# chrischoy/DeepGlobalRegistration

Measured on AMD Instinct MI355X. Metric: pair registrations/sec (FCGF x2 + 1-NN + 6-D inlier net + gate + weighted Procrustes + SE(3) refinement), higher is better.
Workload: dtype f32 results via 2 x f16 split operands (3 f16 MFMA products per MAC, f32 accumulate); k = 1 convs, kNN re-evaluation and registration in exact f32, SVD in f64

## Files before the change

deepglobalregistration_amd/csrc/knn_prefilter.h:

```cpp
#pragma once
#include "knn_common.h"

typedef __attribute__((ext_vector_type(8))) short bf16x8;
typedef __attribute__((ext_vector_type(16))) float f32x16_t;
constexpr float KNN_TAU_C = 8e-5f;
constexpr int KNN_ST = 4;
constexpr int KNN_SLOTS = 32;
#ifndef DGR_KNN_SUB
#define DGR_KNN_SUB 2
#endif
constexpr int KNN_SUB = DGR_KNN_SUB;

__device__ __forceinline__ unsigned short knn_f2bf(float x) {
  uint32_t u = __float_as_uint(x);
  if ((u & 0x7f800000u) == 0x7f800000u) return (unsigned short)((u >> 16) | ((u & 0xffffu) ? 0x40u : 0u));
  u += 0x7fffu + ((u >> 16) & 1u);
  return (unsigned short)(u >> 16);
}
__device__ __forceinline__ float knn_bf2f(unsigned short h) { return __uint_as_float((uint32_t)h << 16); }
__device__ __forceinline__ uint32_t knn_ord(float f) {
  const uint32_t u = __float_as_uint(f);
  return u ^ ((u >> 31) ? 0xffffffffu : 0x80000000u);
}
__device__ __forceinline__ float knn_unord(uint32_t k) {
  return __uint_as_float(k ^ ((k >> 31) ? 0x80000000u : 0xffffffffu));
}
__device__ __forceinline__ int knn_acc_slot(int e, int h) { return (e & 3) + 8 * (e >> 2) + 4 * h; }

template <bool TOPK>
__device__ __forceinline__ int64_t knn_slot_row(int s, int t, int n_tiles) {
  return (int64_t)(TOPK ? (s + t) & 31 : s) * n_tiles + t;
}
template <bool TOPK>
__global__ void __launch_bounds__(256)
    knn_pack_kernel(const float *__restrict__ F0, const float *__restrict__ F1, KnnBatch B,
                    bf16x8 *__restrict__ Qp, bf16x8 *__restrict__ Rp, float *__restrict__ na, float *__restrict__ nb,
                    uint32_t *__restrict__ nb_max, int32_t *__restrict__ fallback) {
  const int pair = blockIdx.y >> 1, side = blockIdx.y & 1;
  const KnnPair d = B.p[pair];
  const int64_t N = side ? d.n1 : d.n0;
  const int64_t n_pad = (N + 31) / 32 * 32;
  const int64_t t = (int64_t)blockIdx.x * blockDim.x + threadIdx.x;
  int64_t row = t >> 2;
  if (row >= n_pad) return;
// ... 9 lines not shown
  for (int e = 0; e < 8; ++e) { hi[e] = 0; lo[e] = 0; }
  if (row < N) {
    const float *src = F + row * 32 + 16 * ch + 8 * g;
    const float4 v0 = *reinterpret_cast<const float4 *>(src), v1 = *reinterpret_cast<const float4 *>(src + 4);
    const float x[8] = {v0.x, v0.y, v0.z, v0.w, v1.x, v1.y, v1.z, v1.w};
#pragma unroll
    for (int e = 0; e < 8; ++e) {
      if (!(fabsf(x[e]) < 1e18f)) fallback[pair] = 1;
      const unsigned short h = knn_f2bf(x[e]);
      const unsigned short l = knn_f2bf(x[e] - knn_bf2f(h));
      hi[e] = (short)knn_f2bf(knn_bf2f(h) * scale);
      lo[e] = (short)knn_f2bf(knn_bf2f(l) * scale);
    }
  }
  const int64_t tile = prow >> 5;
  const int r = (int)(prow & 31);
  packed[(tile * 4 + ch) * 64 + r + 32 * g] = hi;
  packed[(tile * 4 + 2 + ch) * 64 + r + 32 * g] = lo;
  float n = 0.f;
  if (row < N) {
    const float *src = F + row * 32 + 16 * ch + 8 * g;
#pragma unroll
    for (int e = 0; e < 8; ++e) n = fmaf(src[e], src[e], n);
  }
  n += __shfl_xor(n, 1, 64);
  n += __shfl_xor(n, 2, 64);
  if (g == 0 && ch == 0) {
    if (row >= N) n = side ? __builtin_inff() : 0.f;
    else if (side) atomicMax(nb_max + pair, __float_as_uint(n));
    norms[prow] = n;
  }
}

template <bool PASS2, bool TOPK>
__global__ void __launch_bounds__(256, 2)
    knn_mfma_kernel(const bf16x8 *__restrict__ Qp, const bf16x8 *__restrict__ Rp, const float *__restrict__ nbp,
                    KnnBatch B, int splits, int sub_arg, int64_t q_begin, int64_t span, uint32_t *__restrict__ mt,
                    const float *__restrict__ nap, const uint32_t *__restrict__ nb_max,
                    const float *__restrict__ thr_q, int32_t *__restrict__ cand, int32_t *__restrict__ cand_cnt,
                    int slots_arg) {
  __shared__ bf16x8 sA[2][KNN_ST * 4 * 64];
  __shared__ __attribute__((aligned(16))) float sNb[2][KNN_ST * 32];
  const int sub = TOPK ? sub_arg : KNN_SUB, slots = TOPK ? slots_arg : KNN_SLOTS;
  constexpr int NM = TOPK ? 16 : 1;
  const KnnPair d = B.p[blockIdx.z];
  const int n_qblocks = (d.n0 + 31) >> 5, n_rtiles = (d.n1 + 31) >> 5;
  if ((int)blockIdx.x * 16 >= n_qblocks) return;
  const int64_t N0 = d.n0, N1 = d.n1;
  const bf16x8 *Q = Qp + (int64_t)d.qb0 * 256, *R = Rp + (int64_t)d.rt0 * 256;
  const float *nb = nbp + (int64_t)d.rt0 * 32;
  const int64_t qrow0 = d.q0 - q_begin;
  mt += qrow0;
  cand += qrow0 * slots;
  cand_cnt += qrow0;
  const int tid = threadIdx.x;
  const int lane = tid & 63;
  const int wave = __builtin_amdgcn_readfirstlane(tid >> 6);
  const int h = lane >> 5;
  const int qb0 = (blockIdx.x * 4 + wave) * 4;
  bf16x8 bq[4][4];
  float m[4][NM], thr[4];
#pragma unroll
  for (int u = 0; u < 4; ++u) {
    const int qb = min(qb0 + u, n_qblocks - 1);
#pragma unroll
    for (int f = 0; f < 4; ++f) bq[u][f] = Q[((int64_t)qb * 4 + f) * 64 + lane];
#pragma unroll
    for (int e = 0; e < NM; ++e) m[u][e] = __builtin_inff();
    thr[u] = 0.f;
    if constexpr (PASS2) {
      const int64_t q = (int64_t)qb * 32 + (lane & 31);
      const bool live = q < N0 && qb0 + u < n_qblocks;
      if constexpr (TOPK) {
        thr[u] = live ? thr_q[qrow0 + q] : -__builtin_inff();
      } else {
        const float nmax = __uint_as_float(nb_max[blockIdx.z]);
        thr[u] = live ? knn_unord(mt[q]) + KNN_TAU_C * (nap[(int64_t)d.qb0 * 32 + q] + nmax) : -__builtin_inff();
      }
    }
  }
  const int n_stages = (n_rtiles + KNN_ST - 1) / KNN_ST;
  const int sps = (n_stages + splits - 1) / splits;
  const int s_begin = blockIdx.y * sps, s_end = min(n_stages, s_begin + sps);
  const int step = PASS2 ? 1 : sub;
  const int s_first = PASS2 ? s_begin : s_begin + min((int)(blockIdx.y % sub), max(s_end - s_begin - 1, 0));
  if (s_first >= s_end) return;
  bf16x8 pre[KNN_ST];
  float pre_nb = 0.f;
  auto request = [&](int t0) {
#pragma unroll
    for (int j = 0; j < KNN_ST; ++j) pre[j] = R[(int64_t)min(t0 + j, n_rtiles - 1) * 256 + tid];
    if (tid < KNN_ST * 32) pre_nb = nb[(int64_t)min(t0 + (tid >> 5), n_rtiles - 1) * 32 + (tid & 31)];
  };
  auto deposit = [&](int buf) {
#pragma unroll
    for (int j = 0; j < KNN_ST; ++j) sA[buf][j * 256 + tid] = pre[j];
    if (tid < KNN_ST * 32) sNb[buf][tid] = pre_nb;
  };
  request(s_first * KNN_ST);
  deposit(0);
  __syncthreads();
  int buf = 0;
  for (int st = s_first; st < s_end; st += step) {
    const int t0 = st * KNN_ST;
    if (st + step < s_end) request((st + step) * KNN_ST);
#pragma unroll
    for (int j = 0; j < KNN_ST; ++j) {
      const int t = t0 + j;
      if (t >= n_rtiles) break;
      const bf16x8 a0 = sA[buf][(j * 4 + 0) * 64 + lane], a1 = sA[buf][(j * 4 + 1) * 64 + lane];
      const bf16x8 a2 = sA[buf][(j * 4 + 2) * 64 + lane], a3 = sA[buf][(j * 4 + 3) * 64 + lane];
      f32x16_t c0;
#pragma unroll
      for (int g = 0; g < 4; ++g) {
        const float4 v = *reinterpret_cast<const float4 *>(&sNb[buf][j * 32 + 8 * g + 4 * h]);
        c0[4 * g] = v.x; c0[4 * g + 1] = v.y; c0[4 * g + 2] = v.z; c0[4 * g + 3] = v.w;
      }
      f32x16_t acc[4];
#pragma unroll
      for (int u = 0; u < 4; ++u) acc[u] = __builtin_amdgcn_mfma_f32_32x32x16_bf16(a0, bq[u][0], c0, 0, 0, 0);
#pragma unroll
      for (int u = 0; u < 4; ++u) acc[u] = __builtin_amdgcn_mfma_f32_32x32x16_bf16(a1, bq[u][1], acc[u], 0, 0, 0);
#pragma unroll
      for (int u = 0; u < 4; ++u) acc[u] = __builtin_amdgcn_mfma_f32_32x32x16_bf16(a0, bq[u][2], acc[u], 0, 0, 0);
#pragma unroll
      for (int u = 0; u < 4; ++u) acc[u] = __builtin_amdgcn_mfma_f32_32x32x16_bf16(a1, bq[u][3], acc[u], 0, 0, 0);
#pragma unroll
      for (int u = 0; u < 4; ++u) acc[u] = __builtin_amdgcn_mfma_f32_32x32x16_bf16(a2, bq[u][0], acc[u], 0, 0, 0);
#pragma unroll
      for (int u = 0; u < 4; ++u) acc[u] = __builtin_amdgcn_mfma_f32_32x32x16_bf16(a3, bq[u][1], acc[u], 0, 0, 0);
#pragma unroll
      for (int u = 0; u < 4; ++u) {
        if constexpr (!PASS2 && TOPK) {
#pragma unroll
          for (int e = 0; e < 16; ++e) m[u][e] = fminf(m[u][e], acc[u][e]);
        } else {
          float bm = fminf(fminf(acc[u][0], acc[u][1]), fminf(acc[u][2], acc[u][3]));
#pragma unroll
          for (int e = 4; e < 16; e += 4)
            bm = fminf(bm, fminf(fminf(acc[u][e], acc[u][e + 1]), fminf(acc[u][e + 2], acc[u][e + 3])));
          if constexpr (!PASS2) {
            m[u][0] = fminf(m[u][0], bm);
          } else if (!(bm > thr[u])) {
            const int64_t q = (int64_t)(qb0 + u) * 32 + (lane & 31);
#pragma unroll
            for (int e = 0; e < 16; ++e) {
              const int64_t i = knn_slot_row<TOPK>(knn_acc_slot(e, h), t, n_rtiles);
              if (!(acc[u][e] > thr[u]) && q < N0 && i < N1 && qb0 + u < n_qblocks) {
                const int slot = atomicAdd(cand_cnt + q, 1);
                if (slot < slots) cand[q * slots + slot] = (int32_t)(i + d.r0);
              }
            }
          }
        }
      }
    }
    if (st + step < s_end) deposit(buf ^ 1);
    __syncthreads();
    buf ^= 1;
  }
  if constexpr (!PASS2) {
#pragma unroll
    for (int u = 0; u < 4; ++u) {
      const int64_t q = (int64_t)(qb0 + u) * 32 + (lane & 31);
      const bool live = qb0 + u < n_qblocks && q < N0;
      if constexpr (TOPK) {
        if (live) {
#pragma unroll
          for (int e = 0; e < 16; ++e)
            atomicMin(mt + (int64_t)knn_acc_slot(e, h) * span + q, knn_ord(m[u][e]));
        }
      } else {
        const float mm = fminf(m[u][0], __shfl_xor(m[u][0], 32, 64));
        if (lane < 32 && live) atomicMin(mt + q, knn_ord(mm));
      }
    }
  }
}

struct KnnPlan {
  int64_t q_begin, span, n0_max;
  int qb_max, rt_max;
  int qgroups_all;
  bf16x8 *Qp, *Rp;
  float *na, *nb;
  uint32_t *mt;
  float *thr;
  int32_t *qlist, *cand_cnt, *cand;
  uint32_t *nb_max;
  int32_t *fallback, *qcount, *flags;
};

template <bool TOPK>
inline int knn_prefilter_setup(dgr_ctx *ctx, const float *F0, const float *F1, KnnBatch &B, int slots,
                               hipStream_t stream, KnnPlan *plan) {
  KnnPlan &P = *plan;
  DgrArena &arena = ctx->arena;
  int n_qb = 0, n_rt = 0;
  P.qb_max = P.rt_max = P.qgroups_all = 0;
  for (int p = 0; p < B.np; ++p) {
    KnnPair &d = B.p[p];
    d.qb0 = n_qb;
    d.rt0 = n_rt;
    const int qb = (d.n0 + 31) / 32, rt = (d.n1 + 31) / 32;
    n_qb += qb;
    n_rt += rt;
    P.qb_max = std::max(P.qb_max, qb);
    P.rt_max = std::max(P.rt_max, rt);
    P.qgroups_all += (int)dgr_ceil_div(qb, 16);
  }
  P.n0_max = knn_n0_max(B);
  P.span = knn_query_span(B, &P.q_begin);
  const int64_t n_mt = (TOPK ? 32 : 1) * P.span;
  DGR_ALLOC(P.Qp, arena, bf16x8, (int64_t)n_qb * 256);
  DGR_ALLOC(P.Rp, arena, bf16x8, (int64_t)n_rt * 256);
  DGR_ALLOC(P.na, arena, float, (int64_t)n_qb * 32);
  DGR_ALLOC(P.nb, arena, float, (int64_t)n_rt * 32);
  DGR_ALLOC(P.mt, arena, uint32_t, n_mt);
  P.thr = nullptr;
  if (TOPK) DGR_ALLOC(P.thr, arena, float, P.span);
  DGR_ALLOC(P.qlist, arena, int32_t, P.span);
  DGR_ALLOC(P.cand_cnt, arena, int32_t, P.span + 4 * KNN_MAXP);
  DGR_ALLOC(P.cand, arena, int32_t, P.span * slots);
  int32_t *pair_words = P.cand_cnt + P.span;
  P.nb_max = reinterpret_cast<uint32_t *>(pair_words);
  P.fallback = pair_words + KNN_MAXP;
  P.qcount = pair_words + 2 * KNN_MAXP;
  P.flags = pair_words + 3 * KNN_MAXP;
  DGR_HIP_CHECK(hipMemsetAsync(P.cand_cnt, 0, (size_t)(P.span + 4 * KNN_MAXP) * sizeof(int32_t), stream));
  DGR_HIP_CHECK(hipMemsetAsync(P.mt, 0xff, (size_t)n_mt * sizeof(uint32_t), stream));
  dim3 grid((unsigned)dgr_ceil_div((int64_t)std::max(P.qb_max, P.rt_max) * 32 * 4, 256), 2 * B.np);
  knn_pack_kernel<TOPK><<<grid, 256, 0, stream>>>(F0, F1, B, P.Qp, P.Rp, P.na, P.nb, P.nb_max, P.fallback);
  DGR_LAUNCH_CHECK();
  return DGR_OK;
}

template <bool PASS2, bool TOPK>
inline int knn_mfma_launch(dgr_ctx *ctx, const KnnBatch &B, const KnnPlan &P, int sub, int slots, hipStream_t stream) {
  const auto kernel = knn_mfma_kernel<PASS2, TOPK>;
  static int per_cu = 0;
  if (per_cu == 0) {
    int n = 0;
    DGR_HIP_CHECK(hipOccupancyMaxActiveBlocksPerMultiprocessor(&n, kernel, 256, 0));
    per_cu = n < 1 ? 1 : n;
  }
  const int capacity = ctx->num_cus * per_cu;
  const int stages = (int)dgr_ceil_div(P.rt_max, KNN_ST);
  int splits = 1;
  double best_fill = 0.;
  for (int sp = 1; sp <= std::min(16, std::max(1, stages / sub)); ++sp) {
    const int64_t blocks = (int64_t)P.qgroups_all * sp;
    const double fill = (double)blocks / (double)(dgr_ceil_div(blocks, (int64_t)capacity) * capacity);
    if (fill >= best_fill) { best_fill = fill; splits = sp; }
  }
  dim3 grid((unsigned)dgr_ceil_div(P.qb_max, 16), splits, B.np);
  kernel<<<grid, 256, 0, stream>>>(P.Qp, P.Rp, P.nb, B, splits, sub, P.q_begin, P.span, P.mt, P.na, P.nb_max, P.thr,
                                   P.cand, P.cand_cnt, slots);
  DGR_LAUNCH_CHECK();
  return DGR_OK;
}

int knn_list_overflows(const KnnBatch &B, const KnnPlan &P, int slots, hipStream_t stream);
```

deepglobalregistration_amd/_lib.py:

```python
import ctypes as C
import os
import threading

import torch

_HERE = os.path.dirname(os.path.abspath(__file__))
LIB_PATH = os.environ.get('DGR_HIP_LIB') or os.path.join(_HERE, 'lib', 'libdgr_hip.so')

DGR_OK, DGR_EINVAL, DGR_EHIP, DGR_ENOMEM, DGR_ESVD, DGR_EINTERNAL = 0, -1, -2, -3, -4, -5
STATUS_OK, STATUS_LOW_CONFIDENCE, STATUS_SVD_FAILED, STATUS_SAFEGUARD = 0, 1, 2, 3
STATUS_FLAG_ICP_SKIPPED, STATUS_MASK = 0x100, 0xff

c_i32p, c_i64p, c_f32p, c_f64p = (C.POINTER(C.c_int32), C.POINTER(C.c_int64),
                                  C.POINTER(C.c_float), C.POINTER(C.c_double))
vp = C.c_void_p


class WeightDesc(C.Structure):
    _fields_ = [('name', C.c_char_p), ('data', vp), ('numel', C.c_int64)]


class Params(C.Structure):
    _fields_ = [('clip_weight_thresh', C.c_float), ('voxel_size', C.c_float),
                ('inlier_feature_type', C.c_int), ('max_iter', C.c_int),
# ... 31 lines not shown
    'dgr_knn1_l2': (C.c_int, [vp, vp, C.c_int64, vp, C.c_int64, C.c_int, C.c_int, vp, vp, vp]),
    'dgr_knn1_l2_batch': (C.c_int, [vp, vp, c_i64p, vp, c_i64p, C.c_int, C.c_int, C.c_int, vp, vp, vp]),
    'dgr_knn_l2': (C.c_int, [vp, vp, C.c_int64, vp, C.c_int64, C.c_int, C.c_int, C.c_int, vp, vp, vp]),
    'dgr_knn_l2_batch': (C.c_int, [vp, vp, c_i64p, vp, c_i64p, C.c_int, C.c_int, C.c_int, C.c_int, vp, vp,
                                   vp]),
    'dgr_inlier_inputs': (C.c_int, [vp, vp, vp, C.c_int64, vp, vp, C.c_int64, vp, C.c_int, vp, vp, vp]),
    'dgr_sigmoid_clip_sum': (C.c_int, [vp, vp, C.c_int64, C.c_float, vp, c_f64p, vp]),
    'dgr_gather_rows3': (C.c_int, [vp, vp, vp, C.c_int64, vp, vp]),
    'dgr_weighted_procrustes': (C.c_int, [vp, vp, vp, vp, C.c_int64, C.c_float, c_f32p, c_f32p, vp]),
    'dgr_se3_refine': (C.c_int, [vp, vp, vp, vp, C.c_int64, C.c_float, C.c_int, C.c_int, C.c_double,
                                 c_f32p, c_f32p, c_i32p, c_f32p, c_i32p, vp]),
    'dgr_register_batch': (C.c_int, [vp, vp, vp, vp, vp, c_i64p, vp, vp, c_i64p, C.c_int,
                                     C.POINTER(Params), vp, vp, c_f32p, c_i32p, c_f32p, vp]),
    'dgr_register_batch_f64': (C.c_int, [vp, c_f64p, C.c_int64, c_i64p]),
    'dgr_register_batch_output': (C.c_int, [vp, C.c_int, vp, C.c_int64, c_i64p, vp]),
    'dgr_ctx_set_profiling': (C.c_int, [vp, C.c_int]),
    'dgr_icp_point_to_point': (C.c_int, [vp, vp, C.c_int64, vp, C.c_int64, C.c_double, c_f64p, C.c_int, C.c_double,
                                          C.c_double, c_f64p, c_f64p, vp]),
    'dgr_ransac_correspondence': (C.c_int, [vp, vp, vp, C.c_int64, C.c_double, C.c_int64, C.c_uint32, c_f64p, c_f64p, vp]),
    'dgr_ctx_stage_times': (C.c_int, [vp, c_f32p]),
    'dgr_ctx_stage_times_v2': (C.c_int, [vp, c_f32p, C.c_int, C.POINTER(C.c_int)]),
    'dgr_ctx_conv_launches': (C.c_int64, [vp]),
    'dgr_ctx_conv_launch_times': (C.c_int, [vp, c_f32p, c_f32p, C.c_int64, C.POINTER(C.c_int64)]),
    'dgr_ctx_conv_launch_kernel_us': (C.c_int, [vp, c_f32p, C.c_int64, C.POINTER(C.c_int64)]),
    'dgr_ctx_conv_launch_kinds': (C.c_int, [vp, C.c_char_p, C.c_int64, C.POINTER(C.c_int64)]),
    'dgr_radius_pairs_batch': (C.c_int, [vp, vp, c_i64p, vp, c_i64p, C.c_int, c_f64p, C.c_double, C.c_int, vp, vp,
                                         C.c_int64, c_i64p, vp]),
    'dgr_pairs_isin_batch': (C.c_int, [vp, vp, c_i64p, vp, c_i64p, C.c_int, c_i64p, vp, vp]),
    'dgr_validation_counts': (C.c_int, [vp, vp, vp, C.c_float, c_i64p, C.c_int, c_i64p, vp]),
    'dgr_debug_ortho2rotation': (C.c_int, [vp, vp, C.c_int64, vp, vp, vp, vp]),
    'dgr_debug_se3_refine_from': (C.c_int, [vp, vp, vp, vp, C.c_int64, C.c_float, C.c_int, C.c_int, C.c_double,
                                            c_f64p, c_f64p, vp]),
    'dgr_debug_smooth_l1': (C.c_int, [vp, vp, vp, C.c_int64, C.c_float, vp, vp]),
    'dgr_debug_conv_layer': (C.c_int, [vp, vp, C.c_int, vp, vp, C.c_int, C.c_int64, vp, vp]),
}

_lib = None


def load():
    global _lib
    if _lib is not None:
        return _lib
    if not os.path.exists(LIB_PATH):
        raise RuntimeError(
            f'{LIB_PATH} not found: the HIP extension is not built.  Run '
            '`python -c "import __graft_entry__ as g; g.build()"` (or `make -C '
            'deepglobalregistration_amd/csrc`).  There is no CPU fallback.')
    lib = C.CDLL(LIB_PATH)
    for name, (res, args) in SIGNATURES.items():
        fn = getattr(lib, name)
        fn.restype = res
        fn.argtypes = args
    _lib = lib
    return lib


class DgrError(RuntimeError):
    def __init__(self, code, message):
        super().__init__(f'libdgr_hip error {code}: {message}')
        self.code = code


def check(rc):
    if rc == DGR_OK:
        return
# ... 54 lines not shown
```

deepglobalregistration_amd/csrc/dgr_internal.h:

```cpp
#pragma once
#include <hip/hip_runtime.h>
#include <stdint.h>
#include <stdio.h>
#include <stdlib.h>
#include <string>
#include <vector>

#include "../../include/dgr_hip.h"

void dgr_set_error(const char *fmt, ...);

#define DGR_HIP_CHECK(expr)                                                                  \
  do {                                                                                       \
    hipError_t _e = (expr);                                                                  \
    if (_e != hipSuccess) {                                                                  \
      dgr_set_error("%s:%d: %s failed: %s", __FILE__, __LINE__, #expr, hipGetErrorString(_e)); \
      return DGR_EHIP;                                                                       \
    }                                                                                        \
  } while (0)

#define DGR_CHECK(expr)          \
  do {                           \
    int _r = (expr);             \
    if (_r != DGR_OK) return _r; \
// ... 189 lines not shown
                          const int32_t *n_dev, int64_t n_cap, hipStream_t stream);

struct DgrBatchOutputs {
  const void *ptr[5] = {nullptr, nullptr, nullptr, nullptr, nullptr};
  int64_t numel[5] = {0, 0, 0, 0, 0};
  uint64_t generation = 0;
};

struct DgrEventPool {
  std::vector<hipEvent_t> ev;
  size_t used = 0;
  hipEvent_t next();
  void release();
};

struct dgr_ctx {
  int device = 0;
  int num_cus = 256;
  DgrArena arena;
  bool profiling = false;
  float stage_ms[9] = {0, 0, 0, 0, 0, 0, 0, 0, 0};
  int64_t conv_launches = 0;
  DgrBatchOutputs last;
  std::vector<double> last_T64;
  DgrEventPool events;
  std::vector<std::pair<hipEvent_t, hipEvent_t>> conv_spans, gemm_spans, map3_spans, map6_spans;
  std::vector<float> conv_span_ms, gemm_span_ms;
  std::vector<unsigned long long *> conv_clks;
  std::vector<float> conv_clk_us;
  std::vector<const char *> conv_kinds;
  int32_t *flag_dev = nullptr;
  hipEvent_t wait_ev = nullptr;
  long last_wait_ns = 0;
  double batch_ns_per_row = 0;
  unsigned char *pin = nullptr;
  size_t pin_bytes = 0;
  hipStream_t part_stream = nullptr;
  int all_cus = 256;
};

int dgr_ctx_pinned(dgr_ctx *ctx, size_t bytes, unsigned char **out);
int dgr_flag_error(int32_t flag);

int dgr_ctx_wait(dgr_ctx *ctx, hipStream_t stream, long predicted_ns = 0);

int dgr_resunet_forward_impl(dgr_ctx *ctx, dgr_net *net, const int32_t *coords, const float *feats,
                             int64_t N, float *out, hipStream_t stream);
int dgr_ctx_collect_profile(dgr_ctx *ctx);
void dgr_ctx_begin_profile(dgr_ctx *ctx);

int dgr_knn1_batch_impl(dgr_ctx *ctx, const float *F0, const int64_t *off0, const float *F1, const int64_t *off1,
                        int npairs, int C, int squared, int64_t *idx_out, float *dist_out, hipStream_t stream);
int dgr_knn1_impl(dgr_ctx *ctx, const float *F0, int64_t N0, const float *F1, int64_t N1, int C,
                  int squared, int64_t *idx_out, float *dist_out, hipStream_t stream);
int dgr_inlier_inputs_impl(const int32_t *coords0, const float *xyz0, int64_t N0,
                           const int32_t *coords1, const float *xyz1, const int64_t *idx1,
                           int feature_type, int32_t *coords6, float *feats, hipStream_t stream);
int dgr_icp_impl(dgr_ctx *ctx, const float *src, int64_t N0, const float *dst, int64_t N1, double max_dist,
                 const double *T_init, int max_iter, double rel_fitness, double rel_rmse, double *T_out,
                 double *stats_out, hipStream_t stream);
int dgr_ransac_impl(dgr_ctx *ctx, const float *X, const float *Y, int64_t N, double max_dist, int64_t num_hypotheses,
                    uint32_t seed, double *T_out, double *stats_out, hipStream_t stream);
struct DgrIcpJob {
  const float *src = nullptr, *dst = nullptr;
  int64_t N0 = 0, N1 = 0;
  double max_dist = 0;
// ... 30 lines not shown
```

deepglobalregistration_amd/csrc/knn.hip:

```cpp
#include "knn_prefilter.h"

template <int C, int QPT>
__global__ void __launch_bounds__(KNN_THREADS)
    knn1_kernel(const float *__restrict__ F0, const float *__restrict__ F1, KnnBatch B, int splits,
                u64 *__restrict__ best, const int32_t *run_flag, const int32_t *__restrict__ qlist,
                const int32_t *qcount, int64_t q_begin) {
  __shared__ __attribute__((aligned(16))) float tile[KNN_TB * C];
  const KnnPair d = B.p[blockIdx.z];
  if (run_flag && run_flag[blockIdx.z] == 0) return;
  F0 += d.q0 * C;
  F1 += d.r0 * C;
  best += d.q0;
  const int64_t N0 = d.n0, N1 = d.n1;
  if (qlist) qlist += d.q0 - q_begin;
  const int64_t n_q = qlist ? (int64_t)qcount[blockIdx.z] : N0;
  if ((int64_t)blockIdx.x * KNN_THREADS * QPT >= n_q) return;
  const int64_t q0 = ((int64_t)blockIdx.x * KNN_THREADS + threadIdx.x) * QPT;
  const int rows_per_split = (int)(((N1 + splits - 1) / splits + KNN_TB - 1) / KNN_TB) * KNN_TB;
  const int64_t j_begin = (int64_t)blockIdx.y * rows_per_split;
  const int64_t j_end = min(N1, j_begin + rows_per_split);
  if (j_begin >= j_end) return;
  float q[QPT][C];
  int64_t qrow[QPT];
#pragma unroll
// ... 141 lines not shown
    for (int s2 = 32; s2 > 0; s2 >>= 1) {
      const u64 o = __shfl_xor(key, s2, 64);
      key = o < key ? o : key;
    }
    if ((threadIdx.x & 63) == 0) wkey[threadIdx.x >> 6] = key;
    __syncthreads();
    if (threadIdx.x == 0) {
      u64 k3 = wkey[0];
      for (int w = 1; w < 4; ++w) k3 = wkey[w] < k3 ? wkey[w] : k3;
      if (k3 != KNN_KEY_NONE) atomicMin(best + q, k3);
    }
    __syncthreads();
  }
}

__global__ void knn_long_list_flags(const int32_t *__restrict__ qcount, int np, int32_t *__restrict__ flags) {
  if ((int)threadIdx.x < np) flags[threadIdx.x] = qcount[threadIdx.x] > KNN_SCAN_MAX;
}

static int knn_prefiltered(dgr_ctx *ctx, const float *F0, const float *F1, KnnBatch B, u64 *best, hipStream_t stream) {
  KnnPlan P;
  DGR_CHECK(knn_prefilter_setup<false>(ctx, F0, F1, B, KNN_SLOTS, stream, &P));
  DGR_CHECK((knn_mfma_launch<false, false>(ctx, B, P, KNN_SUB, KNN_SLOTS, stream)));
  DGR_CHECK((knn_mfma_launch<true, false>(ctx, B, P, 1, KNN_SLOTS, stream)));
  knn_exact_kernel<<<(int)dgr_ceil_div(P.span, 256), 256, 0, stream>>>(F0, F1, P.cand, P.cand_cnt, P.q_begin,
                                                                      P.q_begin + P.span, best);
  DGR_LAUNCH_CHECK();
  DGR_CHECK(knn_list_overflows(B, P, KNN_SLOTS, stream));
  dim3 grid(KNN_SCAN_SPLITS, B.np);
  knn_query_scan_kernel<<<grid, 256, 0, stream>>>(F0, F1, B, P.q_begin, P.qlist, P.qcount, best);
  knn_long_list_flags<<<1, 64, 0, stream>>>(P.qcount, B.np, P.flags);
  DGR_LAUNCH_CHECK();
  DGR_CHECK(knn_launch<32>(ctx, F0, F1, B, best, P.flags, stream, P.qlist, P.qcount, P.q_begin));
  return knn_launch<32>(ctx, F0, F1, B, best, P.fallback, stream);
}

int dgr_knn1_batch_impl(dgr_ctx *ctx, const float *F0, const int64_t *off0, const float *F1, const int64_t *off1,
                        int npairs, int C, int squared, int64_t *idx_out, float *dist_out, hipStream_t stream) {
  return knn_for_each_table(ctx, off0, off1, npairs, 1, true, stream, [&](const KnnBatch &B, u64 *best) -> int {
    DGR_CHECK(knn_dispatch(
        B, C,
        [&](auto width, const KnnBatch &pairs) {
          return knn_launch<decltype(width)::value>(ctx, F0, F1, pairs, best, nullptr, stream);
        },
        [&](const KnnBatch &pairs) { return knn_prefiltered(ctx, F0, F1, pairs, best, stream); }));
    dim3 grid((unsigned)dgr_ceil_div(knn_n0_max(B), 256), B.np);
    knn1_finish<<<grid, 256, 0, stream>>>(best, B, squared, idx_out, dist_out);
    DGR_LAUNCH_CHECK();
    return DGR_OK;
  });
}

int dgr_knn1_impl(dgr_ctx *ctx, const float *F0, int64_t N0, const float *F1, int64_t N1, int C,
                  int squared, int64_t *idx_out, float *dist_out, hipStream_t stream) {
  const int64_t off0[2] = {0, N0}, off1[2] = {0, N1};
  return dgr_knn1_batch_impl(ctx, F0, off0, F1, off1, 1, C, squared, idx_out, dist_out, stream);
}

extern "C" int dgr_knn1_l2(dgr_ctx *ctx, const float *F0, int64_t N0, const float *F1, int64_t N1, int C,
                           int squared, int64_t *idx_out, float *dist_out, dgr_stream stream) {
  const int64_t off0[2] = {0, N0}, off1[2] = {0, N1};
  DGR_CHECK(knn_enter("dgr_knn1_l2", ctx, F0, F1, idx_out, off0, off1, 1));
  return dgr_knn1_impl(ctx, F0, N0, F1, N1, C, squared, idx_out, dist_out, (hipStream_t)stream);
}

extern "C" int dgr_knn1_l2_batch(dgr_ctx *ctx, const float *F0, const int64_t *off0, const float *F1,
                                 const int64_t *off1, int npairs, int C, int squared, int64_t *idx_out,
                                 float *dist_out, dgr_stream stream) {
  DGR_CHECK(knn_enter("dgr_knn1_l2_batch", ctx, F0, F1, idx_out, off0, off1, npairs));
  return dgr_knn1_batch_impl(ctx, F0, off0, F1, off1, npairs, C, squared, idx_out, dist_out, (hipStream_t)stream);
}
```

deepglobalregistration_amd/ops.py:

```python
import ctypes as C

import numpy as np
import torch

from . import _lib
from ._lib import check, get_ctx, ptr, stream_ptr, vp

F32_EPS = float(np.finfo(np.float32).eps)


def _dev(t):
    if not (torch.is_tensor(t) and t.is_cuda):
        raise ValueError('expected a CUDA(ROCm) tensor')
    return t.device


def _as(t, dtype, device):
    if not torch.is_tensor(t):
        t = torch.as_tensor(np.asarray(t))
    return t.to(device=device, dtype=dtype).contiguous()


def voxelize(xyz, voxel_size, batch_index=0, device='cuda'):
    lib = _lib.load()
# ... 181 lines not shown
    lib = _lib.load()
    dev = _dev(F0)
    F0 = _as(F0, torch.float32, dev)
    F1 = _as(F1, torch.float32, dev)
    if F0.dim() != 2 or F1.dim() != 2 or F0.shape[1] != F1.shape[1]:
        raise ValueError('F0 [N0,C] and F1 [N1,C] must share the feature width')
    N0, N1 = F0.shape[0], F1.shape[0]
    idx = torch.empty(N0, dtype=torch.int64, device=dev)
    dist = torch.empty(N0, dtype=torch.float32, device=dev) if return_distance else None
    check(lib.dgr_knn1_l2(get_ctx(dev), ptr(F0), N0, ptr(F1), N1, F0.shape[1], int(squared), ptr(idx),
                          ptr(dist), stream_ptr(dev.index)))
    return (idx, dist) if return_distance else idx


def knn1_batch(F0, F1, off0, off1, squared=False, return_distance=False):
    lib = _lib.load()
    dev = _dev(F0)
    F0 = _as(F0, torch.float32, dev)
    F1 = _as(F1, torch.float32, dev)
    if F0.dim() != 2 or F1.dim() != 2 or F0.shape[1] != F1.shape[1]:
        raise ValueError('F0 [N0,C] and F1 [N1,C] must share the feature width')
    o0 = np.ascontiguousarray(off0, dtype=np.int64)
    o1 = np.ascontiguousarray(off1, dtype=np.int64)
    if len(o0) != len(o1) or len(o0) < 2 or o0[0] != 0 or o1[0] != 0 or o0[-1] != F0.shape[0] or o1[-1] != F1.shape[0]:
        raise ValueError('off0 / off1 must be [npairs+1] row offsets covering F0 / F1')
    idx = torch.empty(F0.shape[0], dtype=torch.int64, device=dev)
    dist = torch.empty(F0.shape[0], dtype=torch.float32, device=dev) if return_distance else None
    check(lib.dgr_knn1_l2_batch(get_ctx(dev), ptr(F0), o0.ctypes.data_as(_lib.c_i64p), ptr(F1),
                                o1.ctypes.data_as(_lib.c_i64p), len(o0) - 1, F0.shape[1], int(squared), ptr(idx),
                                ptr(dist), stream_ptr(dev.index)))
    return (idx, dist) if return_distance else idx


KNN_MAX_K = 32


def check_knn_k(k):
    if isinstance(k, (bool, np.bool_)) or not isinstance(k, (int, np.integer)):
        raise ValueError(f'knn must be an integer in [1, {KNN_MAX_K}], got {k!r}')
    if not 1 <= int(k) <= KNN_MAX_K:
        raise ValueError(f'knn must be an integer in [1, {KNN_MAX_K}], got {int(k)}')
    return int(k)


def knn(F0, F1, k, squared=False, return_distance=False):
    k = check_knn_k(k)
    lib = _lib.load()
    dev = _dev(F0)
    F0 = _as(F0, torch.float32, dev)
    F1 = _as(F1, torch.float32, dev)
    if F0.dim() != 2 or F1.dim() != 2 or F0.shape[1] != F1.shape[1]:
        raise ValueError('F0 [N0,C] and F1 [N1,C] must share the feature width')
    N0, N1 = F0.shape[0], F1.shape[0]
    idx = torch.empty((N0, k), dtype=torch.int64, device=dev)
    dist = torch.empty((N0, k), dtype=torch.float32, device=dev) if return_distance else None
    check(lib.dgr_knn_l2(get_ctx(dev), ptr(F0), N0, ptr(F1), N1, F0.shape[1], k, int(squared), ptr(idx), ptr(dist),
                         stream_ptr(dev.index)))
    return (idx, dist) if return_distance else idx


def knn_batch(F0, F1, off0, off1, k, squared=False, return_distance=False):
    k = check_knn_k(k)
    lib = _lib.load()
    dev = _dev(F0)
    F0 = _as(F0, torch.float32, dev)
    F1 = _as(F1, torch.float32, dev)
# ... 371 lines not shown
```

include/dgr_hip.h:

```cpp
#ifndef DGR_HIP_H
#define DGR_HIP_H

#include <stdint.h>

#ifdef __cplusplus
extern "C" {
#endif

typedef struct dgr_ctx dgr_ctx;
typedef struct dgr_net dgr_net;
typedef struct dgr_maps dgr_maps;
typedef void *dgr_stream;

enum {
  DGR_OK = 0,
  DGR_EINVAL = -1,
  DGR_EHIP = -2,
  DGR_ENOMEM = -3,
  DGR_ESVD = -4,
  DGR_EINTERNAL = -5
};

enum { DGR_STATUS_OK = 0, DGR_STATUS_LOW_CONFIDENCE = 1, DGR_STATUS_SVD_FAILED = 2,
       DGR_STATUS_SAFEGUARD = 3 ,
// ... 109 lines not shown
                       float *stats_out, dgr_stream stream);
int dgr_register_batch_output(dgr_ctx *ctx, int which, void *dst_dev, int64_t capacity_bytes,
                              int64_t *numel, dgr_stream stream);
int dgr_register_batch_f64(dgr_ctx *ctx, double *T_out, int64_t capacity_pairs, int64_t *npairs);

int dgr_ctx_set_profiling(dgr_ctx *ctx, int enable);
#define DGR_NUM_STAGE_TIMES 9
int dgr_ctx_stage_times_v2(dgr_ctx *ctx, float *times_ms, int capacity, int *n);
int dgr_ctx_stage_times(dgr_ctx *ctx, float *times_ms);
int64_t dgr_ctx_conv_launches(dgr_ctx *ctx);
int dgr_ctx_conv_launch_times(dgr_ctx *ctx, float *times_ms, float *gemm_ms, int64_t capacity, int64_t *n);
int dgr_ctx_conv_launch_kernel_us(dgr_ctx *ctx, float *us, int64_t capacity, int64_t *n);
int dgr_ctx_conv_launch_kinds(dgr_ctx *ctx, char *buf, int64_t capacity, int64_t *n);

int dgr_radius_pairs_batch(dgr_ctx *ctx, const float *xyz0, const int64_t *off0, const float *xyz1,
                           const int64_t *off1, int npairs, const double *T, double radius, int K,
                           int32_t *counts_out, int64_t *pairs_out, int64_t capacity, int64_t *total_out,
                           dgr_stream stream);
int dgr_pairs_isin_batch(dgr_ctx *ctx, const int64_t *pos, const int64_t *pos_off, const int64_t *pred,
                         const int64_t *pred_off, int npairs, const int64_t *M_per_pair, uint8_t *out,
                         dgr_stream stream);
int dgr_validation_counts(dgr_ctx *ctx, const uint8_t *label, const float *weights, float threshold,
                          const int64_t *off, int npairs, int64_t *counts_out, dgr_stream stream);

int dgr_debug_ortho2rotation(dgr_ctx *ctx, const float *p6, int64_t n, const float *grad_R9, float *R9_out,
                             float *grad_p6_out, dgr_stream stream);
int dgr_debug_se3_refine_from(dgr_ctx *ctx, const float *X, const float *Y, const float *w, int64_t N,
                              float quantization_size, int max_iter, int max_break_count,
                              double break_threshold_ratio, const double *state_in, double *state_out,
                              dgr_stream stream);
int dgr_debug_smooth_l1(dgr_ctx *ctx, const float *X, const float *Y, int64_t n, float quantization_size,
                        float *per_point_out, dgr_stream stream);

int dgr_debug_conv_layer(dgr_ctx *ctx, dgr_net *net, int layer, const int32_t *coords, const float *in, int in_relu,
                         int64_t N, float *out, dgr_stream stream);

#ifdef __cplusplus
}
#endif
#endif
```

Before: 386.5.

## Screen kNN pass-2 tiles with a coarse hi-hi product before full refinement

In the second kNN prefilter pass, each 32x32 tile is first scored using only the hi-part bf16 MFMA products. The remaining four correction MFMAs run only when some lane in the wave falls under a widened threshold whose margin bounds the missing lo terms. The goal is to skip most of the split-precision MFMA work for tiles that cannot contain candidates. This adds a per-tile ballot branch and divergent control flow, and correctness depends on the eps bound. An environment variable restores the old path.

```diff
diff --git a/deepglobalregistration_amd/csrc/knn_prefilter.h b/deepglobalregistration_amd/csrc/knn_prefilter.h
--- a/deepglobalregistration_amd/csrc/knn_prefilter.h
+++ b/deepglobalregistration_amd/csrc/knn_prefilter.h
@@ -4,6 +4,7 @@
 typedef __attribute__((ext_vector_type(8))) short bf16x8;
 typedef __attribute__((ext_vector_type(16))) float f32x16_t;
 constexpr float KNN_TAU_C = 8e-5f;
+constexpr float KNN_EPS_C = 1.01f / 128.f;
 constexpr int KNN_ST = 4;
 constexpr int KNN_SLOTS = 32;
 #ifndef DGR_KNN_SUB
@@ -85,7 +86,18 @@
   }
 }
 
-template <bool PASS2, bool TOPK>
+__device__ __forceinline__ float knn_acc_min(const f32x16_t &a) {
+  float bm = fminf(fminf(a[0], a[1]), a[2]);
+#pragma unroll
+  for (int e = 3; e < 15; e += 2) bm = fminf(fminf(bm, a[e]), a[e + 1]);
+  return fminf(bm, a[15]);
+}
+inline bool knn_no_screen() {
+  static const bool off = getenv("DGR_KNN_NO_SCREEN") != nullptr;
+  return off;
+}
+
+template <bool PASS2, bool TOPK, bool SCREEN>
 __global__ void __launch_bounds__(256, 2)
     knn_mfma_kernel(const bf16x8 *__restrict__ Qp, const bf16x8 *__restrict__ Rp, const float *__restrict__ nbp,
                     KnnBatch B, int splits, int sub_arg, int64_t q_begin, int64_t span, uint32_t *__restrict__ mt,
@@ -96,6 +108,7 @@
   __shared__ __attribute__((aligned(16))) float sNb[2][KNN_ST * 32];
   const int sub = TOPK ? sub_arg : KNN_SUB, slots = TOPK ? slots_arg : KNN_SLOTS;
   constexpr int NM = TOPK ? 16 : 1;
+  static_assert(!SCREEN || PASS2, "pass 1 keeps the minima of the full product");
   const KnnPair d = B.p[blockIdx.z];
   const int n_qblocks = (d.n0 + 31) >> 5, n_rtiles = (d.n1 + 31) >> 5;
   if ((int)blockIdx.x * 16 >= n_qblocks) return;
@@ -112,7 +125,7 @@
   const int h = lane >> 5;
   const int qb0 = (blockIdx.x * 4 + wave) * 4;
   bf16x8 bq[4][4];
-  float m[4][NM], thr[4];
+  float m[4][NM], thr[4], thr_hi[4];
 #pragma unroll
   for (int u = 0; u < 4; ++u) {
     const int qb = min(qb0 + u, n_qblocks - 1);
@@ -120,16 +133,18 @@
     for (int f = 0; f < 4; ++f) bq[u][f] = Q[((int64_t)qb * 4 + f) * 64 + lane];
 #pragma unroll
     for (int e = 0; e < NM; ++e) m[u][e] = __builtin_inff();
-    thr[u] = 0.f;
+    thr[u] = thr_hi[u] = 0.f;
     if constexpr (PASS2) {
       const int64_t q = (int64_t)qb * 32 + (lane & 31);
       const bool live = q < N0 && qb0 + u < n_qblocks;
+      const float nmax = __uint_as_float(nb_max[blockIdx.z]);
       if constexpr (TOPK) {
         thr[u] = live ? thr_q[qrow0 + q] : -__builtin_inff();
       } else {
-        const float nmax = __uint_as_float(nb_max[blockIdx.z]);
         thr[u] = live ? knn_unord(mt[q]) + KNN_TAU_C * (nap[(int64_t)d.qb0 * 32 + q] + nmax) : -__builtin_inff();
       }
+      if constexpr (SCREEN)
+        thr_hi[u] = live ? thr[u] + KNN_EPS_C * (nap[(int64_t)d.qb0 * 32 + q] + nmax) : -__builtin_inff();
     }
   }
   const int n_stages = (n_rtiles + KNN_ST - 1) / KNN_ST;
@@ -162,7 +177,6 @@
       const int t = t0 + j;
       if (t >= n_rtiles) break;
       const bf16x8 a0 = sA[buf][(j * 4 + 0) * 64 + lane], a1 = sA[buf][(j * 4 + 1) * 64 + lane];
-      const bf16x8 a2 = sA[buf][(j * 4 + 2) * 64 + lane], a3 = sA[buf][(j * 4 + 3) * 64 + lane];
       f32x16_t c0;
 #pragma unroll
       for (int g = 0; g < 4; ++g) {
@@ -174,36 +188,52 @@
       for (int u = 0; u < 4; ++u) acc[u] = __builtin_amdgcn_mfma_f32_32x32x16_bf16(a0, bq[u][0], c0, 0, 0, 0);
 #pragma unroll
       for (int u = 0; u < 4; ++u) acc[u] = __builtin_amdgcn_mfma_f32_32x32x16_bf16(a1, bq[u][1], acc[u], 0, 0, 0);
-#pragma unroll
-      for (int u = 0; u < 4; ++u) acc[u] = __builtin_amdgcn_mfma_f32_32x32x16_bf16(a0, bq[u][2], acc[u], 0, 0, 0);
-#pragma unroll
-      for (int u = 0; u < 4; ++u) acc[u] = __builtin_amdgcn_mfma_f32_32x32x16_bf16(a1, bq[u][3], acc[u], 0, 0, 0);
-#pragma unroll
-      for (int u = 0; u < 4; ++u) acc[u] = __builtin_amdgcn_mfma_f32_32x32x16_bf16(a2, bq[u][0], acc[u], 0, 0, 0);
-#pragma unroll
-      for (int u = 0; u < 4; ++u) acc[u] = __builtin_amdgcn_mfma_f32_32x32x16_bf16(a3, bq[u][1], acc[u], 0, 0, 0);
-#pragma unroll
-      for (int u = 0; u < 4; ++u) {
-        if constexpr (!PASS2 && TOPK) {
-#pragma unroll
-          for (int e = 0; e < 16; ++e) m[u][e] = fminf(m[u][e], acc[u][e]);
-        } else {
-          float bm = fminf(fminf(acc[u][0], acc[u][1]), fminf(acc[u][2], acc[u][3]));
-#pragma unroll
-          for (int e = 4; e < 16; e += 4)
-            bm = fminf(bm, fminf(fminf(acc[u][e], acc[u][e + 1]), fminf(acc[u][e + 2], acc[u][e + 3])));
-          if constexpr (!PASS2) {
-            m[u][0] = fminf(m[u][0], bm);
-          } else if (!(bm > thr[u])) {
-            const int64_t q = (int64_t)(qb0 + u) * 32 + (lane & 31);
-#pragma unroll
-            for (int e = 0; e < 16; ++e) {
-              const int64_t i = knn_slot_row<TOPK>(knn_acc_slot(e, h), t, n_rtiles);
-              if (!(acc[u][e] > thr[u]) && q < N0 && i < N1 && qb0 + u < n_qblocks) {
-                const int slot = atomicAdd(cand_cnt + q, 1);
-                if (slot < slots) cand[q * slots + slot] = (int32_t)(i + d.r0);
-              }
+      auto refine = [&](f32x16_t &x, int u, const bf16x8 &a2, const bf16x8 &a3) {
+        x = __builtin_amdgcn_mfma_f32_32x32x16_bf16(a0, bq[u][2], x, 0, 0, 0);
+        x = __builtin_amdgcn_mfma_f32_32x32x16_bf16(a1, bq[u][3], x, 0, 0, 0);
+        x = __builtin_amdgcn_mfma_f32_32x32x16_bf16(a2, bq[u][0], x, 0, 0, 0);
+        x = __builtin_amdgcn_mfma_f32_32x32x16_bf16(a3, bq[u][1], x, 0, 0, 0);
+      };
+      auto emit = [&](const f32x16_t &x, int u) {
+        if (!(knn_acc_min(x) > thr[u])) {
+          const int64_t q = (int64_t)(qb0 + u) * 32 + (lane & 31);
+#pragma unroll
+          for (int e = 0; e < 16; ++e) {
+            const int64_t i = knn_slot_row<TOPK>(knn_acc_slot(e, h), t, n_rtiles);
+            if (!(x[e] > thr[u]) && q < N0 && i < N1 && qb0 + u < n_qblocks) {
+              const int slot = atomicAdd(cand_cnt + q, 1);
+              if (slot < slots) cand[q * slots + slot] = (int32_t)(i + d.r0);
             }
+          }
+        }
+      };
+      if constexpr (SCREEN) {
+#pragma unroll
+        for (int u = 0; u < 4; ++u) {
+          if (__builtin_amdgcn_ballot_w64(!(knn_acc_min(acc[u]) > thr_hi[u])) != 0) {
+            refine(acc[u], u, sA[buf][(j * 4 + 2) * 64 + lane], sA[buf][(j * 4 + 3) * 64 + lane]);
+            emit(acc[u], u);
+          }
+        }
+      } else {
+        const bf16x8 a2 = sA[buf][(j * 4 + 2) * 64 + lane], a3 = sA[buf][(j * 4 + 3) * 64 + lane];
+#pragma unroll
+        for (int u = 0; u < 4; ++u) acc[u] = __builtin_amdgcn_mfma_f32_32x32x16_bf16(a0, bq[u][2], acc[u], 0, 0, 0);
+#pragma unroll
+        for (int u = 0; u < 4; ++u) acc[u] = __builtin_amdgcn_mfma_f32_32x32x16_bf16(a1, bq[u][3], acc[u], 0, 0, 0);
+#pragma unroll
+        for (int u = 0; u < 4; ++u) acc[u] = __builtin_amdgcn_mfma_f32_32x32x16_bf16(a2, bq[u][0], acc[u], 0, 0, 0);
+#pragma unroll
+        for (int u = 0; u < 4; ++u) acc[u] = __builtin_amdgcn_mfma_f32_32x32x16_bf16(a3, bq[u][1], acc[u], 0, 0, 0);
+#pragma unroll
+        for (int u = 0; u < 4; ++u) {
+          if constexpr (!PASS2 && TOPK) {
+#pragma unroll
+            for (int e = 0; e < 16; ++e) m[u][e] = fminf(m[u][e], acc[u][e]);
+          } else if constexpr (!PASS2) {
+            m[u][0] = fminf(m[u][0], knn_acc_min(acc[u]));
+          } else {
+            emit(acc[u], u);
           }
         }
       }
@@ -288,9 +318,10 @@
   return DGR_OK;
 }
 
-template <bool PASS2, bool TOPK>
-inline int knn_mfma_launch(dgr_ctx *ctx, const KnnBatch &B, const KnnPlan &P, int sub, int slots, hipStream_t stream) {
-  const auto kernel = knn_mfma_kernel<PASS2, TOPK>;
+template <bool PASS2, bool TOPK, bool SCREEN>
+inline int knn_mfma_launch_as(dgr_ctx *ctx, const KnnBatch &B, const KnnPlan &P, int sub, int slots,
+                              hipStream_t stream) {
+  const auto kernel = knn_mfma_kernel<PASS2, TOPK, SCREEN>;
   static int per_cu = 0;
   if (per_cu == 0) {
     int n = 0;
@@ -313,4 +344,14 @@
   return DGR_OK;
 }
 
+template <bool PASS2, bool TOPK>
+inline int knn_mfma_launch(dgr_ctx *ctx, const KnnBatch &B, const KnnPlan &P, int sub, int slots, hipStream_t stream) {
+  if constexpr (!PASS2) {
+    return knn_mfma_launch_as<PASS2, TOPK, false>(ctx, B, P, sub, slots, stream);
+  } else {
+    return knn_no_screen() ? knn_mfma_launch_as<PASS2, TOPK, false>(ctx, B, P, sub, slots, stream)
+                           : knn_mfma_launch_as<PASS2, TOPK, true>(ctx, B, P, sub, slots, stream);
+  }
+}
+
 int knn_list_overflows(const KnnBatch &B, const KnnPlan &P, int slots, hipStream_t stream);
```

Measured after the change: 392.7, median of 6. 1.6% higher.

## Tighten kNN pass-2 threshold with running bound and batch candidate appends

Applied to the files above, without the earlier changes.

In the kNN prefilter's second pass, each query's threshold is now tightened by a running bound: the best tile minimum seen so far plus the tau margin. This prunes more candidate rows. Hits are buffered per thread in shared memory (up to four per query) and flushed with one atomicAdd per batch instead of one per hit, which cuts atomic traffic on the candidate counters. It also adds a debug entry point that reads back per-pair kNN counters and an overflow check on reference tile counts. The extra shared memory can lower occupancy, and the running bound changes which candidates reach the exact re-evaluation.

```diff
diff --git a/deepglobalregistration_amd/_lib.py b/deepglobalregistration_amd/_lib.py
--- a/deepglobalregistration_amd/_lib.py
+++ b/deepglobalregistration_amd/_lib.py
@@ -87,6 +87,7 @@
     'dgr_debug_se3_refine_from': (C.c_int, [vp, vp, vp, vp, C.c_int64, C.c_float, C.c_int, C.c_int, C.c_double,
                                             c_f64p, c_f64p, vp]),
     'dgr_debug_smooth_l1': (C.c_int, [vp, vp, vp, C.c_int64, C.c_float, vp, vp]),
+    'dgr_debug_knn1_counters': (C.c_int, [vp, c_i32p, C.c_int, C.POINTER(C.c_int), vp]),
     'dgr_debug_conv_layer': (C.c_int, [vp, vp, C.c_int, vp, vp, C.c_int, C.c_int64, vp, vp]),
 }
 
diff --git a/deepglobalregistration_amd/csrc/dgr_internal.h b/deepglobalregistration_amd/csrc/dgr_internal.h
--- a/deepglobalregistration_amd/csrc/dgr_internal.h
+++ b/deepglobalregistration_amd/csrc/dgr_internal.h
@@ -245,6 +245,8 @@
   int32_t *flag_dev = nullptr;
   hipEvent_t wait_ev = nullptr;
   long last_wait_ns = 0;
+  const int32_t *knn_pair_words = nullptr;
+  int knn_pairs = 0;
   double batch_ns_per_row = 0;
   unsigned char *pin = nullptr;
   size_t pin_bytes = 0;
diff --git a/deepglobalregistration_amd/csrc/knn.hip b/deepglobalregistration_amd/csrc/knn.hip
--- a/deepglobalregistration_amd/csrc/knn.hip
+++ b/deepglobalregistration_amd/csrc/knn.hip
@@ -197,11 +197,14 @@
   knn_long_list_flags<<<1, 64, 0, stream>>>(P.qcount, B.np, P.flags);
   DGR_LAUNCH_CHECK();
   DGR_CHECK(knn_launch<32>(ctx, F0, F1, B, best, P.flags, stream, P.qlist, P.qcount, P.q_begin));
+  ctx->knn_pair_words = P.fallback;
+  ctx->knn_pairs = B.np;
   return knn_launch<32>(ctx, F0, F1, B, best, P.fallback, stream);
 }
 
 int dgr_knn1_batch_impl(dgr_ctx *ctx, const float *F0, const int64_t *off0, const float *F1, const int64_t *off1,
                         int npairs, int C, int squared, int64_t *idx_out, float *dist_out, hipStream_t stream) {
+  ctx->knn_pairs = 0;
   return knn_for_each_table(ctx, off0, off1, npairs, 1, true, stream, [&](const KnnBatch &B, u64 *best) -> int {
     DGR_CHECK(knn_dispatch(
         B, C,
@@ -235,3 +238,19 @@
   DGR_CHECK(knn_enter("dgr_knn1_l2_batch", ctx, F0, F1, idx_out, off0, off1, npairs));
   return dgr_knn1_batch_impl(ctx, F0, off0, F1, off1, npairs, C, squared, idx_out, dist_out, (hipStream_t)stream);
 }
+
+extern "C" int dgr_debug_knn1_counters(dgr_ctx *ctx, int32_t *counters_out, int max_pairs, int *npairs_out,
+                                       dgr_stream stream) {
+  DGR_REQUIRE(ctx && counters_out && npairs_out && max_pairs >= 0, "dgr_debug_knn1_counters: bad argument");
+  DGR_HIP_CHECK(hipSetDevice(ctx->device));
+  DGR_HIP_CHECK(hipStreamSynchronize((hipStream_t)stream));
+  const int np = std::min(ctx->knn_pairs, max_pairs);
+  int32_t words[2 * KNN_MAXP];
+  if (np > 0) DGR_HIP_CHECK(hipMemcpy(words, ctx->knn_pair_words, sizeof(words), hipMemcpyDeviceToHost));
+  for (int p = 0; p < np; ++p) {
+    counters_out[2 * p] = words[p];
+    counters_out[2 * p + 1] = words[KNN_MAXP + p];
+  }
+  *npairs_out = np;
+  return DGR_OK;
+}
diff --git a/deepglobalregistration_amd/csrc/knn_prefilter.h b/deepglobalregistration_amd/csrc/knn_prefilter.h
--- a/deepglobalregistration_amd/csrc/knn_prefilter.h
+++ b/deepglobalregistration_amd/csrc/knn_prefilter.h
@@ -10,6 +10,10 @@
 #define DGR_KNN_SUB 2
 #endif
 constexpr int KNN_SUB = DGR_KNN_SUB;
+constexpr int KNN_HITS = 4;
+#ifndef DGR_KNN_RUNNING_BOUND
+#define DGR_KNN_RUNNING_BOUND 1
+#endif
 
 __device__ __forceinline__ unsigned short knn_f2bf(float x) {
   uint32_t u = __float_as_uint(x);
@@ -94,6 +98,8 @@
                     int slots_arg) {
   __shared__ bf16x8 sA[2][KNN_ST * 4 * 64];
   __shared__ __attribute__((aligned(16))) float sNb[2][KNN_ST * 32];
+  constexpr bool LISTS = PASS2 && !TOPK;
+  __shared__ int32_t sHit[LISTS ? 4 * KNN_HITS * 256 : 1];
   const int sub = TOPK ? sub_arg : KNN_SUB, slots = TOPK ? slots_arg : KNN_SLOTS;
   constexpr int NM = TOPK ? 16 : 1;
   const KnnPair d = B.p[blockIdx.z];
@@ -112,9 +118,14 @@
   const int h = lane >> 5;
   const int qb0 = (blockIdx.x * 4 + wave) * 4;
   bf16x8 bq[4][4];
-  float m[4][NM], thr[4];
+  float m[4][NM], thr[4], tau[4];
+  int n_hit[4];
+  bool live_q[4];
 #pragma unroll
   for (int u = 0; u < 4; ++u) {
+    tau[u] = 0.f;
+    n_hit[u] = 0;
+    live_q[u] = false;
     const int qb = min(qb0 + u, n_qblocks - 1);
 #pragma unroll
     for (int f = 0; f < 4; ++f) bq[u][f] = Q[((int64_t)qb * 4 + f) * 64 + lane];
@@ -129,6 +140,8 @@
       } else {
         const float nmax = __uint_as_float(nb_max[blockIdx.z]);
         thr[u] = live ? knn_unord(mt[q]) + KNN_TAU_C * (nap[(int64_t)d.qb0 * 32 + q] + nmax) : -__builtin_inff();
+        tau[u] = live ? KNN_TAU_C * (nap[(int64_t)d.qb0 * 32 + q] + nmax) : 0.f;
+        live_q[u] = live;
       }
     }
   }
@@ -138,6 +151,15 @@
   const int step = PASS2 ? 1 : sub;
   const int s_first = PASS2 ? s_begin : s_begin + min((int)(blockIdx.y % sub), max(s_end - s_begin - 1, 0));
   if (s_first >= s_end) return;
+  auto flush = [&](int u, int64_t q) {
+    if constexpr (LISTS) {
+      const int n = n_hit[u];
+      const int slot = atomicAdd(cand_cnt + q, n);
+      for (int k = 0; k < n; ++k)
+        if (slot + k < slots) cand[q * slots + slot + k] = sHit[(u * KNN_HITS + k) * 256 + tid];
+      n_hit[u] = 0;
+    }
+  };
   bf16x8 pre[KNN_ST];
   float pre_nb = 0.f;
   auto request = [&](int t0) {
@@ -194,14 +216,35 @@
             bm = fminf(bm, fminf(fminf(acc[u][e], acc[u][e + 1]), fminf(acc[u][e + 2], acc[u][e + 3])));
           if constexpr (!PASS2) {
             m[u][0] = fminf(m[u][0], bm);
-          } else if (!(bm > thr[u])) {
-            const int64_t q = (int64_t)(qb0 + u) * 32 + (lane & 31);
-#pragma unroll
-            for (int e = 0; e < 16; ++e) {
-              const int64_t i = knn_slot_row<TOPK>(knn_acc_slot(e, h), t, n_rtiles);
-              if (!(acc[u][e] > thr[u]) && q < N0 && i < N1 && qb0 + u < n_qblocks) {
-                const int slot = atomicAdd(cand_cnt + q, 1);
-                if (slot < slots) cand[q * slots + slot] = (int32_t)(i + d.r0);
+          } else if constexpr (TOPK) {
+            if (!(bm > thr[u])) {
+              const int64_t q = (int64_t)(qb0 + u) * 32 + (lane & 31);
+#pragma unroll
+              for (int e = 0; e < 16; ++e) {
+                const int64_t i = knn_slot_row<TOPK>(knn_acc_slot(e, h), t, n_rtiles);
+                if (!(acc[u][e] > thr[u]) && q < N0 && i < N1 && qb0 + u < n_qblocks) {
+                  const int slot = atomicAdd(cand_cnt + q, 1);
+                  if (slot < slots) cand[q * slots + slot] = (int32_t)(i + d.r0);
+                }
+              }
+            }
+          } else {
+            if constexpr (DGR_KNN_RUNNING_BOUND) thr[u] = fminf(thr[u], fminf(bm, __shfl_xor(bm, 32, 64)) + tau[u]);
+            if (!(bm > thr[u]) && live_q[u]) {
+              uint32_t hits = 0;
+#pragma unroll
+              for (int e = 0; e < 16; ++e) hits |= (uint32_t)(!(acc[u][e] > thr[u])) << e;
+              const int64_t q = (int64_t)(qb0 + u) * 32 + (lane & 31);
+              const int row0 = 4 * h * n_rtiles + t;
+              while (hits) {
+                const int e = __builtin_ctz(hits);
+                hits &= hits - 1;
+                const int i = ((e & 3) + 8 * (e >> 2)) * n_rtiles + row0;
+                if (i < d.n1) {
+                  if (n_hit[u] == KNN_HITS) flush(u, q);
+                  sHit[(u * KNN_HITS + n_hit[u]) * 256 + tid] = i + (int32_t)d.r0;
+                  ++n_hit[u];
+                }
               }
             }
           }
@@ -211,6 +254,11 @@
     if (st + step < s_end) deposit(buf ^ 1);
     __syncthreads();
     buf ^= 1;
+  }
+  if constexpr (LISTS) {
+#pragma unroll
+    for (int u = 0; u < 4; ++u)
+      if (n_hit[u] > 0) flush(u, (int64_t)(qb0 + u) * 32 + (lane & 31));
   }
   if constexpr (!PASS2) {
 #pragma unroll
@@ -255,7 +303,8 @@
     KnnPair &d = B.p[p];
     d.qb0 = n_qb;
     d.rt0 = n_rt;
-    const int qb = (d.n0 + 31) / 32, rt = (d.n1 + 31) / 32;
+    const int qb = (int)(((int64_t)d.n0 + 31) / 32), rt = (int)(((int64_t)d.n1 + 31) / 32);
+    DGR_REQUIRE((int64_t)rt * 32 <= (int64_t)INT32_MAX, "find_knn: pair %d: more than 2^31 - 32 references", p);
     n_qb += qb;
     n_rt += rt;
     P.qb_max = std::max(P.qb_max, qb);
diff --git a/deepglobalregistration_amd/ops.py b/deepglobalregistration_amd/ops.py
--- a/deepglobalregistration_amd/ops.py
+++ b/deepglobalregistration_amd/ops.py
@@ -237,6 +237,15 @@
     return (idx, dist) if return_distance else idx
 
 
+def debug_knn1_counters(device=None):
+    import ctypes as C
+    dev = torch.device(device) if device is not None else torch.device('cuda', torch.cuda.current_device())
+    out = (C.c_int32 * 64)()
+    n = C.c_int(0)
+    check(_lib.load().dgr_debug_knn1_counters(get_ctx(dev), out, 32, C.byref(n), stream_ptr(dev.index)))
+    return [(int(out[2 * p]), int(out[2 * p + 1])) for p in range(n.value)]
+
+
 KNN_MAX_K = 32
 
 
diff --git a/include/dgr_hip.h b/include/dgr_hip.h
--- a/include/dgr_hip.h
+++ b/include/dgr_hip.h
@@ -165,6 +165,8 @@
 int dgr_debug_smooth_l1(dgr_ctx *ctx, const float *X, const float *Y, int64_t n, float quantization_size,
                         float *per_point_out, dgr_stream stream);
 
+int dgr_debug_knn1_counters(dgr_ctx *ctx, int32_t *counters_out, int max_pairs, int *npairs_out, dgr_stream stream);
+
 int dgr_debug_conv_layer(dgr_ctx *ctx, dgr_net *net, int layer, const int32_t *coords, const float *in, int in_relu,
                          int64_t N, float *out, dgr_stream stream);
 
```

After: 389.5 before, 393.2 after, median of 6. About the same (+1.0%).
